# tmtlakmal/acme

Measured on AMD Instinct MI355X. Metric: learner transitions/sec (sample+step) at batch 512, 1/2/4/8 MI355X, higher is better.
Workload: dtype f32 (2xf16 split planes, 3 MFMA terms); 1 GPU; dqn_nature_cnn_prioritized_replay (BASELINE configs[1]); global_batch=512, batch_per_gpu=512, replay_slots=1000000, replay_slots_per_gpu=1000000, obs=uint8[84,84,4], num_actions=18, sampler=prioritized(alpha=0.6), IS beta=0.2, prefetch_size=4, parallelism=dp1

## Files before the change

### acme_amd/_lib.py

```python

from __future__ import annotations

import ctypes
import os
import threading

import torch

_HERE = os.path.dirname(os.path.abspath(__file__))
LIB_PATH = os.environ.get("ACME_LIB_PATH") or os.path.join(_HERE, "libacme_hip.so")

ACME_OK = 0
ACME_ERR_INVALID = -1
ACME_ERR_HIP = -2
ACME_ERR_EMPTY = -3
ACME_ERR_OOM = -4

SEMANTICS_TF = 0
SEMANTICS_JAX = 1

MATMUL_F32 = 0
MATMUL_X6 = 1

MAX_FIELDS = 16
# ... 196 lines not shown
    "acme_replay_update_priorities_gated": (c_i32, [c_vp, c_vp, c_vp, c_i64, c_vp, c_vp]),
    "acme_replay_size": (c_i64, [c_vp]),
    "acme_replay_capacity": (c_i64, [c_vp]),
    "acme_replay_debug_leaves": (c_i32, [c_vp, ctypes.POINTER(c_vp), ctypes.POINTER(c_vp),
                                         ctypes.POINTER(c_vp)]),
    "acme_replay_debug_level": (c_i32, [c_vp, c_i32, ctypes.POINTER(c_vp),
                                        ctypes.POINTER(c_i64), ctypes.POINTER(c_i32)]),
    "acme_replay_storage": (c_i32, [c_vp, c_i32, ctypes.POINTER(c_vp)]),
    "acme_replay_inserted": (c_i64, [c_vp]),
    "acme_replay_restore": (c_i32, [c_vp, c_i64, c_vp]),
    "acme_demo_store_create": (c_i32, [c_i64, c_vp, c_i32, c_vp, c_i64, ctypes.POINTER(c_vp)]),
    "acme_demo_store_destroy": (c_i32, [c_vp]),
    "acme_demo_store_upload": (c_i32, [c_vp, ctypes.POINTER(c_vp)]),
    "acme_demo_mix": (c_i32, [c_vp, c_f64, c_i32, c_f32, c_u64, c_u64, c_i64,
                              ctypes.POINTER(c_vp), c_vp, c_vp, c_vp, c_vp, c_vp, c_vp]),
    "acme_seq_demo_mix": (c_i32, [c_vp, c_f64, c_i64, c_i64, c_u64, c_u64, c_i64,
                                  ctypes.POINTER(c_vp), c_i32, c_vp, c_vp, c_vp, c_vp, c_vp,
                                  c_vp, c_vp, c_vp]),
    "acme_dqn_num_params": (c_i64, [c_vp]),
    "acme_dqn_plane_overflow": (c_i32, [c_vp, ctypes.POINTER(c_i32), c_i32]),
    "acme_dqn_verdict_timeouts": (c_i32, [c_vp, ctypes.POINTER(c_i64)]),
    "acme_dqn_update_rider_launches": (c_i64, [c_vp]),
    "acme_dqn_fused_x2_launches": (c_i64, [c_vp]),
    "acme_dqn_skip_word": (c_i32, [c_vp, ctypes.POINTER(c_vp)]),
    "acme_dqn_set_reissue": (c_i32, [c_vp, c_i32]),
    "acme_dqn_verdicts_issued": (c_i64, [c_vp]),
    "acme_dqn_step_verdict": (c_i32, [c_vp, c_i64, ctypes.POINTER(c_i32)]),
    "acme_dqn_set_data_parallel_gate": (c_i32, [c_vp, c_i32]),
    "acme_dqn_dense_grads_ready": (c_i32, [c_vp, c_vp]),
    "acme_dqn_dp_init": (c_i32, [c_vp, c_vp, c_i32]),
    "acme_dqn_dp_step": (c_i32, [c_vp, ctypes.POINTER(TransitionBatch), ctypes.POINTER(DQNOutputs),
                                 c_vp]),
    "acme_nccl_get_unique_id": (c_i32, [c_vp]),
    "acme_nccl_comm_init": (c_i32, [c_vp, c_i32, c_i32, ctypes.POINTER(c_vp)]),
    "acme_nccl_comm_destroy": (c_i32, [c_vp]),
    "acme_dqn_forward_backward": (c_i32, [c_vp, ctypes.POINTER(TransitionBatch),
                                          ctypes.POINTER(DQNOutputs), c_vp]),
    "acme_dqn_apply": (c_i32, [c_vp, c_vp]),
    "acme_dqn_forward_backward_stage": (c_i32, [c_vp, ctypes.POINTER(TransitionBatch),
                                                ctypes.POINTER(DQNOutputs), c_i32, c_vp]),
    "acme_dqn_grad_split": (c_i32, [c_vp, ctypes.POINTER(c_i64)]),
    "acme_dqn_step": (c_i32, [c_vp, ctypes.POINTER(TransitionBatch), ctypes.POINTER(DQNOutputs),
                              c_vp]),
    "acme_dqn_step_update": (c_i32, [c_vp, ctypes.POINTER(TransitionBatch),
                                     ctypes.POINTER(DQNOutputs), c_vp, c_vp, c_vp, c_vp]),
    "acme_dqn_q_values": (c_i32, [c_vp, c_vp, c_i64, c_i32, c_vp, c_vp]),
# ... 180 lines not shown
```

### acme_amd/csrc/dqn.hip

```cpp
#include <hip/hip_runtime.h>

#include <algorithm>
#include <cmath>
#include <cstring>
#include <string>
#include <vector>

#include "common.h"
#include "conv.h"
#include "rescale.h"
#include "conv_p3.h"
#include "gemm.h"
#include "gemm_p3.h"
#include "gemm_x6.h"
#include "kernels.h"
#include "launch.h"
#include "learner_common.h"
#include "plane_guard.h"
#include "prio_update.h"
#include "profiler.h"
#include "rccl_dyn.h"
#include "torso.h"

using namespace acme;
using namespace acme::conv;
using acme::gemm::launch_gemm;

namespace {

using torso::G1;
constexpr int kFlat = torso::kFlat;
constexpr int kHidden = 512;
constexpr int kObsBytes = 84 * 84 * 4;

struct Layer {
  int in = 0, out = 0;
  int w = -1, b = -1;
// ... 57 lines not shown
  uint16_t *wpl = nullptr, *tpl = nullptr;
  uint16_t* frames = nullptr;
  StepState step;
  hipStream_t side = nullptr;
  hipEvent_t ev[4] = {nullptr, nullptr, nullptr, nullptr};
  float* slab2 = nullptr;
  float* side_slab = nullptr;
  float* tslab = nullptr;
  bool target_dirty = true;
  torso::Plane x1p{}, x2p{}, x3p{}, t1p{}, t2p{}, t3p{}, dzhp{}, dz3p{}, dz2p{}, dz1p{};
  hipEvent_t ev_dense = nullptr;
  void* dp_comm = nullptr;
  int dp_world = 0;
  hipStream_t dp_stream = nullptr;
  hipEvent_t dp_ev[4] = {nullptr, nullptr, nullptr, nullptr};
  double* dp_gmin = nullptr;
  double* loss_part = nullptr;
  bool single_stream = false;
  bool single_role = false;
  bool bk32 = false;
  bool update_rider = true;
  int64_t rider_launches = 0;
  bool head_fuse = true;
  int fuse_x2 = torso::kFuseX2Default;
  int64_t fused_x2_launches = 0;
  bool frames_u8 = true;
  int64_t seq = 0;
  uint32_t* host_verdicts = nullptr;
  uint32_t verdict_seq = 0;
  bool sticky = false;
  bool dp_gate = false;
  int64_t dp_gate_index = -1;
};

namespace {

enum {
  kScX1, kScX2, kScX3, kScT1, kScT2, kScT3, kScDzh, kScDz3, kScDz2, kScDz1,
  kScTransient,
  kScParams = kScTransient, kScTarget,
  kScCount
};
constexpr int64_t kParamAmaxPeriod = 8;
constexpr int kVerdictRing = 64;

int add_tensor(acme_dqn* l, const std::string& name, std::initializer_list<int64_t> shape) {
// ... 3 lines not shown
}

inline torso::Plane WP(const acme_dqn* l, uint16_t* base, int t) {
  return torso::Plane{base + l->tensors[t].offset, l->flat,
                      l->scales + (base == l->tpl ? kScTarget : kScParams)};
}
int convert_frames(acme_dqn* l, const void* obs_a, const void* obs_b, int split, int rows,
                   hipStream_t st) {
  ACME_PROF("frames_f16", st, 0.0, 3.0 * (double)rows * kObsBytes);
  return launch_frames_f16(static_cast<const uint8_t*>(obs_a), static_cast<const uint8_t*>(obs_b),
                           split, rows, kObsBytes, l->frames, st);
}
bool use_p3(const acme_dqn* l) { return l->p3_capable && gemm::use_x6(); }
Gate step_gate(const acme_dqn* l) {
  Gate q;
  q.g = l->guard;
  q.par = (int)(l->seq & 1);
  if (l->dp_gate) q.dp = l->grads + l->dp_gate_index;
  return q;
}
hipStream_t side_stream(const acme_dqn* l) { return prof::enabled() ? nullptr : l->side; }

constexpr int kFcFwdSplits = 8;
constexpr int kHeadFwdSplits = 16;
constexpr int kHeadBwdSplits = 8;

int64_t slab_floats_needed(int B, int A) {
  return std::max<int64_t>({torso::wgrad_slab_floats(), (int64_t)kFcFwdSplits * 2 * B * 2 * kHidden,
                            (int64_t)kHeadFwdSplits * 2 * B * (A + 1),
                            (int64_t)kHeadBwdSplits * (2 * kHidden + 1) * (A + 1)});
}

int slab_reduce(const float* slab, int splits, int64_t count, float* out0, int64_t split_at,
                float* out1, const float* bias, int ncols, int relu, const char* name,
                hipStream_t st) {
  ACME_PROF(name, st, 0.0, 4.0 * (double)(splits + 1) * (double)count);
  return launch_slab_reduce(slab, splits, count, out0, split_at, out1, bias, ncols, relu, st);
}

int adam_range(acme_dqn* l, int64_t off, int64_t n, const Gate& gate, const AdamTail& tail,
               hipStream_t st) {
  const bool jax = l->cfg.semantics == ACME_SEMANTICS_JAX;
  const bool p3 = l->p3_capable;
  return launch_adam(l->params + off, l->grads + off, l->m + off, l->v + off, n,
                     l->cfg.learning_rate, l->cfg.adam_beta1, l->cfg.adam_beta2,
                     l->cfg.adam_epsilon, 0, p3 ? l->wpl + off : nullptr, l->flat, st, jax ? 1 : 0,
// ... 50 lines not shown
  return head_forward(l, prm, rows, hid, q, st);
}

template <int BM>
int fc_fwd_gemm(const acme_dqn* l, const char* name, P3DenseFwd p, int splits,
                hipStream_t st) {
  if (l->single_role) ACME_P3_GEMM(name, BM, 128, 2, 2, 32, p, splits);
  else ACME_P3WS_GEMM(name, BM, 128, 2, 2, 32, p, splits);
  return ACME_OK;
}

int nature_forward_p3(acme_dqn* l, const float* prm, uint16_t* wpl, const torso::Frames& frames,
                      int rows, const torso::Plane& x1, const torso::Plane& x2,
                      const torso::Plane& x3, float* hid, float* q, hipStream_t st,
                      float* slab = nullptr, int keep_x1 = -1, bool defer_head = false,
                      int keep_x2 = -1) {
  if (!slab) slab = l->slab;
  int rc = torso::forward_p3(torso_pweights(l, prm, wpl), frames, rows, torso::PActs{x1, x2, x3}, st, keep_x1, l->bk32, keep_x2);
  if (rc != ACME_OK) return rc;
  {
    P3DenseFwd p;
    const bool tall = rows > 512;
    const bool ttall = rows == 512 && !defer_head;
    const int splits = kFcFwdSplits;
    p.M = rows; p.N = 2 * kHidden; p.K = kFlat; p.k_chunk = chunk_for(kFlat, splits);
    p.a_src = SRC(x3, (int64_t)rows * kFlat); p.ldx = kFlat;
    p.b_src = SRC(WP(l, wpl, l->t_fcw), (int64_t)kFlat * 2 * kHidden); p.slab = slab;
    if (tall) p.stamps = l->stamps;
    rc = tall || ttall ? fc_fwd_gemm<256>(l, ttall ? "fc_fwd_target" : "fc_fwd", p, splits, st)
                       : fc_fwd_gemm<128>(l, "fc_fwd", p, splits, st);
    if (rc != ACME_OK) return rc;
    if (defer_head && l->head_fuse &&
        dqn_head_loss_dz_fusable(kHidden, l->cfg.num_actions, splits, P(l, prm, l->t_vw),
                                 P(l, prm, l->t_aw), P(l, prm, l->t_fcb))) {
      l->step.head_deferred = true;
      l->step.head_splits = splits;
      return ACME_OK;
    }
    ACME_PROF("fc_head_fwd", st, 0.0, 4.0 * (double)rows * 2 * kHidden * (splits + 1));
    return launch_fc_head_forward(slab, splits, rows, kHidden, P(l, prm, l->t_fcb),
                                  P(l, prm, l->t_vw), P(l, prm, l->t_vb), P(l, prm, l->t_aw),
                                  P(l, prm, l->t_ab), l->cfg.num_actions, hid, q, st);
  }
}

template <class In>
int mlp_layer(acme_dqn* l, const float* prm, const Layer& L, const void* a, const void* b,
              int split, int rows, float* y, hipStream_t st) {
  const bool vec = L.in % 4 == 0 && L.out % 4 == 0;
  if (vec) {
    DenseFwd<true, In> p;
    p.M = rows; p.N = L.out; p.K = L.in; p.k_chunk = L.in;
    p.x = static_cast<const typename In::T*>(a); p.x2 = static_cast<const typename In::T*>(b);
// ... 76 lines not shown
                     s.upd_n >= 1 && s.upd_n <= kUpdateRiderMax;
  if (rider) {
    if (plan.after) ACME_HIP_TRY(hipStreamWaitEvent(st, plan.after, 0));
    const RescaleJob job = take_step_rescale(l, true);
    if ((rc = replay_update_prepare(plan.replay, plan.keys, s.upd_prio, s.upd_n, step_gate(l), st,
                                    &job, kUpdateRiderBlocks, &upd)) != ACME_OK)
      return rc;
    l->rider_launches += 1;
    s.update_issued = true;
  }
  rc = torso::backward_p3_conv1(g, s.cur_frames, B, l->dz1p, l->slab, st, sd,
                                rider ? &upd : nullptr);
  if (rider) replay_update_release(plan.replay);
  if (rc != ACME_OK) return rc;
  if (write_back && !rider) {
    s.update_issued = true;
    if (plan.after) ACME_HIP_TRY(hipStreamWaitEvent(st, plan.after, 0));
    const RescaleJob job = take_step_rescale(l, true);
    if ((rc = replay_update_priorities_gated(plan.replay, plan.keys, s.upd_prio, s.upd_n,
                                             step_gate(l), st, &job)) != ACME_OK)
      return rc;
  }
  return torso::backward_p3_join(st, sd);
}

int nature_backward(acme_dqn* l, const StepPlan& plan, const void* o_tm1, int B,
                    hipStream_t st_main, bool join_dense) {
  StepState& s = l->step;
  hipStream_t st = st_main;
  const float* prm = l->params;
  float* gr = l->grads;
  const int A = l->cfg.num_actions;
  const bool p3 = use_p3(l);
  int rc;
  bool loss_sum = false;
  const LossArgs la = s.pending_la;
  if (p3 && s.loss_pending && s.head_deferred) {
    s.loss_pending = s.head_deferred = false;
    loss_sum = true;
    s.loss_nparts = B;
    ACME_PROF("head_loss_dz", st, 0.0, 4.0 * (double)2 * B * 2 * kHidden * (s.head_splits + 1));
    rc = launch_dqn_head_loss_dz(la, l->slab, s.head_splits, kHidden, P(l, prm, l->t_fcb),
                                 P(l, prm, l->t_vw), P(l, prm, l->t_vb), P(l, prm, l->t_aw),
                                 P(l, prm, l->t_ab), l->hid, l->dzhp.p, l->dzhp.stride,
                                 l->dzhp.sc, st,
                                 l->stamps && B <= 4096 ? l->stamps + (int64_t)5 * 4096 * 8 : nullptr);
    if (rc != ACME_OK) return rc;
  } else if (p3 && s.loss_pending) {
    s.loss_pending = false;
    loss_sum = la.loss_part != nullptr;
    s.loss_nparts = dqn_loss_head_dz_blocks(B, kHidden);
    ACME_PROF("loss_head_dz", st, 0.0, 0.0);
    rc = launch_dqn_loss_head_dz(la, l->hid, kHidden, P(l, prm, l->t_vw),
                                 P(l, prm, l->t_aw), l->dzhp.p, l->dzhp.stride, l->dzhp.sc, st);
    if (rc != ACME_OK) return rc;
  } else {
    ACME_PROF("head_dz", st, 0.0, 0.0);
    rc = p3 ? launch_head_dz_planes(l->hid, l->g, l->a_cache, B, kHidden, A, P(l, prm, l->t_vw),
                                    P(l, prm, l->t_aw), l->dzhp.p, l->dzhp.stride, l->dzhp.sc, st)
            : launch_duel_head_dz(l->hid, l->g, l->a_cache, B, kHidden, A, P(l, prm, l->t_vw),
                                  P(l, prm, l->t_aw), l->dzh, st);
    if (rc != ACME_OK) return rc;
  }
  const bool fork = p3 && side_stream(l);
  float* hslab = fork ? l->side_slab : l->slab;
  if (fork) {
    ACME_HIP_TRY(hipEventRecord(l->ev[2], st_main));
    ACME_HIP_TRY(hipStreamWaitEvent(l->side, l->ev[2], 0));
    st = l->side;
  }
  if (p3 && plan.replay) {
    s.upd_prio = la.prio;
    s.upd_n = B;
  }
  const bool sum_in_scatter = loss_sum;
  {
    DuelHeadWgrad p;
    p.M = 2 * kHidden; p.N = A + 1; p.K = B; p.k_chunk = chunk_for(B, kHeadBwdSplits);
    p.A = A; p.h = l->hid; p.g = l->g; p.act = l->a_cache; p.slab = hslab;
    ACME_GEMM("head_wgrad", 64, 32, 2, 1, 16, 1, p, kHeadBwdSplits);
    ACME_PROF("head_wgrad_scatter", st, 0.0, 0.0);
    rc = launch_duel_head_grad_scatter(
        hslab, kHeadBwdSplits, kHidden, A, Pm(l, gr, l->t_vw), Pm(l, gr, l->t_vb),
        Pm(l, gr, l->t_aw), Pm(l, gr, l->t_ab), st, sum_in_scatter ? la.loss_part : nullptr,
        s.loss_nparts, la.mean_over, la.loss);
    if (rc != ACME_OK) return rc;
  }
  if (p3) {
    {
      P3DenseWgrad p;
      p.M = kFlat; p.N = 2 * kHidden; p.K = B; p.k_chunk = B;
      p.a_src = SRC(l->x3p, (int64_t)B * kFlat); p.ldx = kFlat;
      p.b_src = SRC(l->dzhp, (int64_t)B * 2 * kHidden); p.out = Pm(l, gr, l->t_fcw);
      p.bias_out = Pm(l, gr, l->t_fcb);
      ACME_P3_GEMM("fc_wgrad", 128, 128, 2, 2, 16, p, 1);
    }
    if (fork) {
      ACME_HIP_TRY(hipEventRecord(l->ev[3], l->side));
      st = st_main;
    }
    {
      P3DenseDgrad p;
      p.M = B; p.N = kFlat; p.K = 2 * kHidden; p.k_chunk = p.K;
      p.a_src = SRC(l->dzhp, (int64_t)B * 2 * kHidden);
      p.b_src = SRC(WP(l, l->wpl, l->t_fcw), (int64_t)kFlat * 2 * kHidden); p.xprev = CP(l->x3p);
      p.ldx = kFlat; p.dx = PP(l->dz3p);
      if (l->single_role) ACME_P3G_GEMM("fc_dgrad", 128, 128, 2, 2, 32, 3, p, 1);
      else ACME_P3WS_GEMM("fc_dgrad", 128, 128, 2, 2, 32, p, 1);
    }
    if (fork && join_dense) ACME_HIP_TRY(hipStreamWaitEvent(st_main, l->ev[3], 0));
    if (fork) s.dense_ev = l->ev[3];
    return ACME_OK;
  }
  {
    DenseWgrad<true> p;
    p.M = kFlat; p.N = 2 * kHidden; p.K = B; p.k_chunk = B;
    p.x = l->x3; p.ldx = kFlat; p.dz = l->dzh; p.out = Pm(l, gr, l->t_fcw);
    p.bias_out = Pm(l, gr, l->t_fcb);
    ACME_GEMM("fc_wgrad", 128, 128, 2, 2, 16, 1, p, 1);
  }
  {
    DenseDgrad<true> p;
    p.M = B; p.N = kFlat; p.K = 2 * kHidden; p.k_chunk = p.K;
    p.dz = l->dzh; p.w = P(l, prm, l->t_fcw); p.xprev = l->x3; p.ldx = kFlat; p.dx = l->dz3;
    ACME_GEMM("fc_dgrad", 64, 128, 2, 2, 16, 1, p, 1);
  }
  return ACME_OK;
}

template <class In>
int mlp_wgrad(acme_dqn* l, const Layer& L, const void* x, const float* dz, int B, float* dw,
              float* db, hipStream_t st) {
  if (L.in % 4 == 0 && L.out % 4 == 0) {
    DenseWgrad<true, In> p;
    p.M = L.in; p.N = L.out; p.K = B; p.k_chunk = B;
    p.x = static_cast<const typename In::T*>(x); p.ldx = L.in; p.dz = dz; p.out = dw;
// ... 67 lines not shown
}

extern "C" {

int acme_dqn_create(const acme_dqn_config* cfg, acme_dqn** out) {
  ACME_CHECK_ARG(cfg && out, "null argument");
  ACME_CHECK_ARG(cfg->num_actions >= 1 && cfg->num_actions <= 63, "num_actions must be in [1, 63]");
  ACME_CHECK_ARG(cfg->max_batch >= 1 && cfg->max_batch <= 65536, "max_batch must be in [1, 65536]");
  ACME_CHECK_ARG(cfg->network == ACME_NET_NATURE_DQN || cfg->network == ACME_NET_MLP,
                 "unknown network kind %d", cfg->network);
  ACME_CHECK_ARG(cfg->obs_dtype == ACME_OBS_U8_SCALED || cfg->obs_dtype == ACME_OBS_F32,
                 "unknown observation dtype %d", cfg->obs_dtype);
  ACME_CHECK_ARG(cfg->huber_loss_parameter >= 0.f, "quadratic_linear_boundary must be >= 0.");
  ACME_CHECK_ARG(cfg->target_update_period >= 1, "target_update_period must be >= 1");
  ACME_CHECK_ARG(cfg->semantics == ACME_SEMANTICS_TF || cfg->semantics == ACME_SEMANTICS_JAX,
                 "unknown learner semantics %d", cfg->semantics);
  acme_dqn* l = new acme_dqn();
  l->cfg = *cfg;
  l->single_stream = tune_variant("SIDE") == 1;
  l->single_role = tune_variant("WSN") == 1;
  l->bk32 = tune_variant("BK32") == 1;
  l->update_rider = tune_variant("UPDATE_RIDER", kUpdateRiderDefault) != 0;
  l->head_fuse = tune_variant("HEAD_FUSE", 1) != 0;
  l->fuse_x2 = tune_variant("FUSE_X2", torso::kFuseX2Default) & 3;
  l->stamps_on = tune_variant("STAMPS") == 1;
  const int A = cfg->num_actions;
  const int B = cfg->max_batch;
  int rc = ACME_OK;
  auto fail = [&](int code) {
    acme_dqn_destroy(l);
    return code;
  };
  if ((rc = guard_create(l)) != ACME_OK) return fail(rc);
  if (hipHostMalloc(reinterpret_cast<void**>(&l->host_verdicts), kVerdictRing * sizeof(uint32_t),
                    hipHostMallocCoherent | hipHostMallocMapped) != hipSuccess)
    return fail((set_error("step guard allocation failed"), ACME_ERR_HIP));
  for (int i = 0; i < kVerdictRing; ++i) l->host_verdicts[i] = 0xFFFFFFFFu;
  if (cfg->network == ACME_NET_NATURE_DQN) {
    l->t_c1w = add_tensor(l, "atari_torso/conv2_d/w", {8, 8, 4, 32});
    l->t_c1b = add_tensor(l, "atari_torso/conv2_d/b", {32});
    l->t_c2w = add_tensor(l, "atari_torso/conv2_d_1/w", {4, 4, 32, 64});
    l->t_c2b = add_tensor(l, "atari_torso/conv2_d_1/b", {64});
    l->t_c3w = add_tensor(l, "atari_torso/conv2_d_2/w", {3, 3, 64, 64});
    l->t_c3b = add_tensor(l, "atari_torso/conv2_d_2/b", {64});
    l->t_fcw = add_tensor(l, "duelling_q_network/hidden/w", {kFlat, 2 * kHidden});
    l->t_fcb = add_tensor(l, "duelling_q_network/hidden/b", {2 * kHidden});
// ... 172 lines not shown
int acme_dqn_guard_state(acme_dqn* l, int64_t* out4) {
  ACME_CHECK_ARG(l && out4 && l->guard, "null argument");
  StepGuard g;
  if (int rc = read_guard(l, &g)) return rc;
  out4[0] = g.applied;
  out4[1] = g.skipped;
  out4[2] = g.last;
  out4[3] = g.qv;
  return ACME_OK;
}

int acme_dqn_verdict_timeouts(acme_dqn* l, int64_t* out) {
  ACME_CHECK_ARG(l && out, "null argument");
  *out = 0;
  if (!l->guard) return ACME_OK;
  StepGuard g;
  if (int rc = read_guard(l, &g)) return rc;
  *out = g.vtimeout;
  return ACME_OK;
}

int64_t acme_dqn_update_rider_launches(const acme_dqn* l) { return l ? l->rider_launches : 0; }
int64_t acme_dqn_fused_x2_launches(const acme_dqn* l) { return l ? l->fused_x2_launches : 0; }

int acme_dqn_set_reissue(acme_dqn* l, int32_t enable) {
  ACME_CHECK_ARG(l, "null learner");
  l->sticky = enable != 0 && l->p3_capable;
  return ACME_OK;
}

int64_t acme_dqn_verdicts_issued(const acme_dqn* l) { return l ? (int64_t)l->verdict_seq : 0; }

int acme_dqn_step_verdict(const acme_dqn* l, int64_t seq, int32_t* state) {
  ACME_CHECK_ARG(l && state && seq >= 0, "bad argument");
  *state = -1;
  if (!l->host_verdicts || seq >= (int64_t)l->verdict_seq) return ACME_OK;
  ACME_CHECK_ARG(seq + kVerdictRing >= (int64_t)l->verdict_seq,
                 "verdict %lld is older than the ring's %d", (long long)seq, kVerdictRing);
  const uint32_t v =
      __atomic_load_n(l->host_verdicts + (seq & (kVerdictRing - 1)), __ATOMIC_ACQUIRE);
  if ((v >> 1) == ((uint32_t)seq & 0x7fffffffu)) *state = (int32_t)(v & 1u);
  return ACME_OK;
}

int acme_dqn_set_applied_steps(acme_dqn* l, int64_t n) {
  ACME_CHECK_ARG(l && l->guard && n >= 0, "bad argument");
// ... 518 lines not shown
```

### acme_amd/csrc/kernels.hip

```cpp
#include "kernels.h"
#include "rescale.h"

#include "conv.h"
#include "gemm_p3.h"
#include "gemm_x6.h"

#include <hip/hip_runtime.h>

#include <algorithm>
#include <cmath>

#include "common.h"
#include "detmath.h"

namespace acme {
namespace {

__global__ void __launch_bounds__(256) duel_head_finish_kernel(const float* __restrict__ slab,
                                                               int splits, int rows, int A,
                                                               const float* __restrict__ bv,
                                                               const float* __restrict__ ba,
                                                               float* __restrict__ q) {
  const int lane = threadIdx.x & 63;
  const int row = blockIdx.x * 4 + (threadIdx.x >> 6);
  if (row >= rows) return;
  const int N = A + 1;
  float* qr = q + (size_t)row * A;
  float v = 0.f;
  for (int s = 0; s < splits; ++s) v += slab[((size_t)s * rows + row) * N + A];
  v += bv[0];
  float first = 0.f, part = 0.f;
  for (int j = lane; j < A; j += 64) {
    float acc = 0.f;
    for (int s = 0; s < splits; ++s) acc += slab[((size_t)s * rows + row) * N + j];
    acc += ba[j];
    if (j == lane) {
// ... 113 lines not shown
                                    float* __restrict__ dzh, uint16_t* __restrict__ planes,
                                    int64_t pstride, gemm::PScale* sc) {
  const int64_t i = (int64_t)blockIdx.x * blockDim.x + threadIdx.x;
  if (i >= (int64_t)B * 2 * H) return;
  const int b = (int)(i / (2 * H));
  const int k = (int)(i - (int64_t)b * 2 * H);
  const float gb = g[b];
  float d;
  if (k < H) {
    d = gb * wv[k];
  } else {
    const float* row = wa + (size_t)(k - H) * A;
    const float inv_a = 1.f / (float)A;
    const int ab = a[b];
    float s = 0.f;
    for (int j = 0; j < A; ++j) s = fmaf(gb * ((j == ab ? 1.f : 0.f) - inv_a), row[j], s);
    d = s;
  }
  const float z = h[i] > 0.f ? d : 0.f;
  if (planes) gemm::Planes{planes, pstride, sc}.put(i, z);
  else dzh[i] = z;
}

__device__ __forceinline__ void loss_sum_block(const double* __restrict__ part, int64_t n,
                                               int mean_over, float* __restrict__ loss) {
  __shared__ double red[4];
  const int tid = threadIdx.x, lane = tid & 63, wave = tid >> 6;
  double s = 0.0;
  for (int64_t i = tid; i < n; i += 256) s += part[i];
#pragma unroll
  for (int o = 32; o > 0; o >>= 1) s += __shfl_xor(s, o, 64);
  if (lane == 0) red[wave] = s;
  __syncthreads();
  if (tid == 0) loss[0] = (float)((((red[0] + red[1]) + red[2]) + red[3]) / (double)mean_over);
}

__global__ void __launch_bounds__(256) duel_head_grad_scatter_kernel(
    const float* __restrict__ slab, int splits, int H, int A, float* __restrict__ dwv,
    float* __restrict__ dbv, float* __restrict__ dwa, float* __restrict__ dba,
    const double* __restrict__ part, int64_t nparts, int mean_over, float* __restrict__ loss) {
  if (part && blockIdx.x == gridDim.x - 1) {
    loss_sum_block(part, nparts, mean_over, loss);
    return;
  }
  const int N = A + 1;
  const int64_t count = (int64_t)(2 * H + 1) * N;
  const int64_t e = (int64_t)blockIdx.x * blockDim.x + threadIdx.x;
  if (e >= count) return;
  const int k = (int)(e / N), n = (int)(e - (int64_t)k * N);
  const bool value_w = k < H && n == A, adv_w = k >= H && k < 2 * H && n < A, bias = k == 2 * H;
  if (!(value_w || adv_w || bias)) return;
  float s = 0.f;
  for (int sp = 0; sp < splits; ++sp) s += slab[(size_t)sp * count + e];
  if (value_w) dwv[k] = s;
  else if (adv_w) dwa[(size_t)(k - H) * A + n] = s;
  else if (n == A) dbv[0] = s;
  else dba[n] = s;
}

__global__ void onehot_dq_kernel(const float* __restrict__ g, const int32_t* __restrict__ a,
                                 int B, int A, float* __restrict__ dz) {
  const int i = blockIdx.x * blockDim.x + threadIdx.x;
  if (i >= B * A) return;
  const int b = i / A, j = i - b * A;
  dz[i] = j == a[b] ? g[b] : 0.f;
// ... 1282 lines not shown
         reinterpret_cast<uintptr_t>(fcb) % 16 == 0;
}

int launch_dqn_head_loss_dz(const LossArgs& args, const float* slab, int splits, int H,
                            const float* fcb, const float* wv, const float* bv, const float* wa,
                            const float* ba, float* hid, uint16_t* planes, int64_t pstride,
                            gemm::PScale* sc, hipStream_t st, uint64_t* stamps) {
  ACME_CHECK_ARG(dqn_head_loss_dz_fusable(H, args.A, splits, wv, wa, fcb) && args.loss_part &&
                     planes && sc && args.B >= 1,
                 "bad fused head / loss / head dZ arguments");
  if (splits == 8)
    dqn_head_loss_dz_kernel<8, 18><<<(unsigned)args.B, 256, 0, st>>>(args, slab, fcb, wv, bv, wa, ba,
                                                                   hid, planes, pstride, sc, stamps);
  else
    dqn_head_loss_dz_kernel<4, 18><<<(unsigned)args.B, 256, 0, st>>>(args, slab, fcb, wv, bv, wa, ba,
                                                                   hid, planes, pstride, sc, stamps);
  ACME_LAUNCH_CHECK();
  return ACME_OK;
}

__global__ void __launch_bounds__(256) dqn_loss_sum_kernel(const double* __restrict__ part,
                                                           int64_t n, int mean_over,
                                                           float* __restrict__ loss) {
  loss_sum_block(part, n, mean_over, loss);
}

int launch_dqn_loss_sum(const double* part, int64_t n, int mean_over, float* loss, hipStream_t st) {
  ACME_CHECK_ARG(part && loss && n >= 1 && mean_over >= 1, "bad loss sum args");
  dqn_loss_sum_kernel<<<1, 256, 0, st>>>(part, n, mean_over, loss);
  ACME_LAUNCH_CHECK();
  return ACME_OK;
}

int launch_dqn_loss_head_dz(const LossArgs& args, const float* h, int H, const float* wv,
                            const float* wa, uint16_t* planes, int64_t pstride, gemm::PScale* sc,
                            hipStream_t st) {
  ACME_CHECK_ARG(args.B >= 1 && args.A >= 1 && h && wv && wa && planes && sc,
                 "bad loss / head dZ args");
  const int per = 2 * H / 8;
  ACME_CHECK_ARG(H % 8 == 0 && per >= 32 && 256 % per == 0, "hidden size %d: 2H/8 must divide 256", H);
  ACME_CHECK_ARG(reinterpret_cast<uintptr_t>(wv) % 16 == 0, "wv must be 16-byte aligned");
  const int64_t nb = ceil_div((int64_t)args.B * per, 256);
  dqn_loss_head_dz_kernel<<<(unsigned)(args.loss_part ? nb : nb + 1), 256, 0, st>>>(
      args, h, H, wv, wa, planes, pstride, sc);
  ACME_LAUNCH_CHECK();
  return ACME_OK;
}
// ... 296 lines not shown
```

### acme_amd/native.py

```python

from __future__ import annotations

import ctypes
from typing import Dict, List, Optional, Sequence, Tuple

import numpy as np
import torch

from acme_amd import _lib
from acme_amd._lib import check, lib, ptr, stream_ptr

SAMPLER_UNIFORM = 0
SAMPLER_PRIORITIZED = 1


class NativeReplay:

    def __init__(self, capacity: int, field_bytes: Sequence[int], prioritized: bool,
                 priority_exponent: float = 0.6, seed: int = 1234, device=None):
        _lib.require_gpu()
        if len(field_bytes) > _lib.MAX_FIELDS:
            raise ValueError(f"at most {_lib.MAX_FIELDS} flattened fields per item")
        cfg = _lib.ReplayConfig()
        cfg.capacity = int(capacity)
# ... 585 lines not shown
        self.semantics = semantics
        self.network = network
        self.num_actions = int(num_actions)
        self.max_batch = int(max_batch)
        self._create(cfg, device)
        self.num_params = int(lib().acme_dqn_num_params(self._h))
        d = self.device
        self.loss = torch.zeros(1, dtype=torch.float32, device=d)
        self.td_error = torch.zeros(max_batch, dtype=torch.float32, device=d)
        self.priorities = torch.zeros(max_batch, dtype=torch.float64, device=d)

    def guard_state(self) -> Dict[str, int]:
        g = super().guard_state()
        t = ctypes.c_int64()
        check(lib().acme_dqn_verdict_timeouts(self._h, ctypes.byref(t)), "dqn verdict_timeouts")
        g["verdict_timeouts"] = int(t.value)
        return g

    def update_rider_launches(self) -> int:
        return int(lib().acme_dqn_update_rider_launches(self._h))

    def fused_x2_launches(self) -> int:
        return int(lib().acme_dqn_fused_x2_launches(self._h))

    @property
    def skip_word(self) -> Optional[int]:
        p = ctypes.c_void_p()
        check(lib().acme_dqn_skip_word(self._h, ctypes.byref(p)), "dqn skip_word")
        return p.value

    def set_reissue(self, enable: bool) -> None:
        check(lib().acme_dqn_set_reissue(self._h, 1 if enable else 0), "dqn set_reissue")

    @property
    def verdicts_issued(self) -> int:
        return int(lib().acme_dqn_verdicts_issued(self._h))

    def step_verdict(self, seq: int) -> Optional[bool]:
        v = ctypes.c_int32(-1)
        check(lib().acme_dqn_step_verdict(self._h, int(seq), ctypes.byref(v)), "dqn step_verdict")
        return None if v.value < 0 else bool(v.value)

    def set_data_parallel_gate(self, enable: bool) -> None:
        check(lib().acme_dqn_set_data_parallel_gate(self._h, 1 if enable else 0), "dqn dp gate")

    def _batch(self, o_tm1, a_tm1, r_t, d_t, o_t, probabilities, global_min_probability=None,
# ... 532 lines not shown
```

### include/acme_hip.h

```cpp
#ifndef ACME_HIP_H_
#define ACME_HIP_H_

#include <stdint.h>

#ifdef __cplusplus
extern "C" {
#endif

typedef enum acme_status {
  ACME_OK = 0,
  ACME_ERR_INVALID = -1,
  ACME_ERR_HIP = -2,
  ACME_ERR_EMPTY = -3,
  ACME_ERR_OOM = -4
} acme_status;

const char* acme_last_error(void);

int acme_tune_set(const char* key, int32_t value);
const char* acme_version(void);
const char* acme_target_arch(void);

int acme_event_create(void** ev);
int acme_event_destroy(void* ev);
// ... 177 lines not shown

int acme_dqn_create(const acme_dqn_config* cfg, acme_dqn** out);
int acme_dqn_destroy(acme_dqn* l);
int64_t acme_dqn_num_params(const acme_dqn* l);
int64_t acme_dqn_flat_size(const acme_dqn* l);
int32_t acme_dqn_num_tensors(const acme_dqn* l);
int acme_dqn_tensor_info(const acme_dqn* l, int32_t i, int64_t* offset, int64_t* numel,
                         int32_t* ndim, int64_t* shape4, const char** name);

int acme_dqn_bind(acme_dqn* l, float* params, float* target, float* grads, float* adam_m,
                  float* adam_v);
int acme_dqn_params_changed(acme_dqn* l);
int acme_dqn_plane_overflow(acme_dqn* l, int32_t* overflow, int32_t reset);
int64_t acme_dqn_skipped_steps(const acme_dqn* l);
int acme_dqn_guard_state(acme_dqn* l, int64_t* out4);
int acme_dqn_set_applied_steps(acme_dqn* l, int64_t n);
int acme_dqn_skip_word(const acme_dqn* l, const uint32_t** out);
int acme_dqn_set_data_parallel_gate(acme_dqn* l, int32_t enable);
int acme_dqn_set_reissue(acme_dqn* l, int32_t enable);
int acme_dqn_verdict_timeouts(acme_dqn* l, int64_t* out);
int64_t acme_dqn_verdicts_issued(const acme_dqn* l);
int64_t acme_dqn_update_rider_launches(const acme_dqn* l);
int64_t acme_dqn_fused_x2_launches(const acme_dqn* l);
int acme_dqn_step_verdict(const acme_dqn* l, int64_t seq, int32_t* state);
int acme_dqn_scale_state(const acme_dqn* l, float* out, int32_t capacity, int32_t* count);
int acme_dqn_set_scale_state(acme_dqn* l, const float* in, int32_t count);

typedef struct acme_transition_batch {
  const void* o_tm1;
  const int32_t* a_tm1;
  const float* r_t;
  const float* d_t;
  const void* o_t;
  const double* probabilities;
  int64_t batch;
  const double* global_min_probability;
  int64_t mean_over;
  const uint16_t* obs_f16;
  void* inputs_event;
} acme_transition_batch;

typedef struct acme_dqn_outputs {
  float* loss;
  float* td_error;
  double* priorities;
  float* q_tm1;
// ... 379 lines not shown
```

Measured before the change: 1.152 million transitions/s.

## Fuse dueling head weight-gradient into fc_wgrad GEMM as rider blocks; split tall fc_fwd fewer ways

Introduces a HeadWgradRider that computes the dueling head's value/advantage weight and bias gradients, plus the loss sum, in extra workgroups appended to the fc_wgrad P3 GEMM launch. This replaces the separate split-K head_wgrad GEMM and its scatter kernel. The head backward and fc_dgrad are also restructured into helpers, and the whole dense wgrad chain now runs on the side stream. Separately, tall deferred-head forward passes use 4 K-splits with 128-wide tiles instead of 8 splits with 256-wide tiles. Both paths are on by default behind tune flags, and the rider adds a register-heavy 18-accumulator path inside the GEMM kernel.

After: 1.158 million transitions/s (median of 6 runs). No clear change (+0.5%).

```diff
diff --git a/acme_amd/_lib.py b/acme_amd/_lib.py
--- a/acme_amd/_lib.py
+++ b/acme_amd/_lib.py
@@ -242,6 +242,7 @@
     "acme_dqn_verdict_timeouts": (c_i32, [c_vp, ctypes.POINTER(c_i64)]),
     "acme_dqn_update_rider_launches": (c_i64, [c_vp]),
     "acme_dqn_fused_x2_launches": (c_i64, [c_vp]),
+    "acme_dqn_head_rider_launches": (c_i64, [c_vp]),
     "acme_dqn_skip_word": (c_i32, [c_vp, ctypes.POINTER(c_vp)]),
     "acme_dqn_set_reissue": (c_i32, [c_vp, c_i32]),
     "acme_dqn_verdicts_issued": (c_i64, [c_vp]),
diff --git a/acme_amd/csrc/dqn.hip b/acme_amd/csrc/dqn.hip
--- a/acme_amd/csrc/dqn.hip
+++ b/acme_amd/csrc/dqn.hip
@@ -13,6 +13,7 @@
 #include "gemm.h"
 #include "gemm_p3.h"
 #include "gemm_x6.h"
+#include "head_rider.h"
 #include "kernels.h"
 #include "launch.h"
 #include "learner_common.h"
@@ -116,6 +117,9 @@
   bool update_rider = true;
   int64_t rider_launches = 0;
   bool head_fuse = true;
+  bool fc_split4 = true;
+  bool head_rider = true;
+  int64_t head_rider_launches = 0;
   int fuse_x2 = torso::kFuseX2Default;
   int64_t fused_x2_launches = 0;
   bool frames_u8 = true;
@@ -165,6 +169,7 @@
 hipStream_t side_stream(const acme_dqn* l) { return prof::enabled() ? nullptr : l->side; }
 
 constexpr int kFcFwdSplits = 8;
+constexpr int kFcFwdSplitsTall = 4;
 constexpr int kHeadFwdSplits = 16;
 constexpr int kHeadBwdSplits = 8;
 
@@ -261,13 +266,15 @@
     P3DenseFwd p;
     const bool tall = rows > 512;
     const bool ttall = rows == 512 && !defer_head;
-    const int splits = kFcFwdSplits;
+    const bool half = tall && defer_head && l->fc_split4;
+    const int splits = half ? kFcFwdSplitsTall : kFcFwdSplits;
     p.M = rows; p.N = 2 * kHidden; p.K = kFlat; p.k_chunk = chunk_for(kFlat, splits);
     p.a_src = SRC(x3, (int64_t)rows * kFlat); p.ldx = kFlat;
     p.b_src = SRC(WP(l, wpl, l->t_fcw), (int64_t)kFlat * 2 * kHidden); p.slab = slab;
     if (tall) p.stamps = l->stamps;
-    rc = tall || ttall ? fc_fwd_gemm<256>(l, ttall ? "fc_fwd_target" : "fc_fwd", p, splits, st)
-                       : fc_fwd_gemm<128>(l, "fc_fwd", p, splits, st);
+    rc = (tall && !half) || ttall
+             ? fc_fwd_gemm<256>(l, ttall ? "fc_fwd_target" : "fc_fwd", p, splits, st)
+             : fc_fwd_gemm<128>(l, "fc_fwd", p, splits, st);
     if (rc != ACME_OK) return rc;
     if (defer_head && l->head_fuse &&
         dqn_head_loss_dz_fusable(kHidden, l->cfg.num_actions, splits, P(l, prm, l->t_vw),
@@ -390,6 +397,58 @@
       return rc;
   }
   return torso::backward_p3_join(st, sd);
+}
+
+int head_wgrad(acme_dqn* l, const LossArgs& la, const double* part, int B, float* hslab,
+               hipStream_t st) {
+  const int A = l->cfg.num_actions;
+  float* gr = l->grads;
+  DuelHeadWgrad p;
+  p.M = 2 * kHidden; p.N = A + 1; p.K = B; p.k_chunk = chunk_for(B, kHeadBwdSplits);
+  p.A = A; p.h = l->hid; p.g = l->g; p.act = l->a_cache; p.slab = hslab;
+  ACME_GEMM("head_wgrad", 64, 32, 2, 1, 16, 1, p, kHeadBwdSplits);
+  ACME_PROF("head_wgrad_scatter", st, 0.0, 0.0);
+  return launch_duel_head_grad_scatter(hslab, kHeadBwdSplits, kHidden, A, Pm(l, gr, l->t_vw),
+                                       Pm(l, gr, l->t_vb), Pm(l, gr, l->t_aw), Pm(l, gr, l->t_ab),
+                                       st, part, l->step.loss_nparts, la.mean_over, la.loss);
+}
+
+int dense_wgrads_p3(acme_dqn* l, const StepPlan& plan, const LossArgs& la, const double* part,
+                    int B, float* hslab, hipStream_t st) {
+  float* gr = l->grads;
+  HeadWgradArgs ra;
+  ra.h = l->hid; ra.g = l->g; ra.act = l->a_cache;
+  ra.B = B; ra.A = l->cfg.num_actions; ra.H = kHidden;
+  ra.dwv = Pm(l, gr, l->t_vw); ra.dbv = Pm(l, gr, l->t_vb);
+  ra.dwa = Pm(l, gr, l->t_aw); ra.dba = Pm(l, gr, l->t_ab);
+  ra.part = part; ra.nparts = l->step.loss_nparts; ra.mean_over = la.mean_over; ra.loss = la.loss;
+  const bool rider = l->head_rider && !plan.calibrating && HeadWgradRider::fits(ra);
+  int rc;
+  if (!rider && (rc = head_wgrad(l, la, part, B, hslab, st)) != ACME_OK) return rc;
+  P3DenseWgrad p;
+  p.M = kFlat; p.N = 2 * kHidden; p.K = B; p.k_chunk = B;
+  p.a_src = SRC(l->x3p, (int64_t)B * kFlat); p.ldx = kFlat;
+  p.b_src = SRC(l->dzhp, (int64_t)B * 2 * kHidden); p.out = Pm(l, gr, l->t_fcw);
+  p.bias_out = Pm(l, gr, l->t_fcb);
+  if (rider) {
+    l->head_rider_launches += 1;
+    ACME_LAUNCH_GEMM("fc_wgrad", ACME_MNK_FLOPS(p), gemm::p3_peak_tflops<decltype(p)>(),
+                     (gemm::launch_gemm_p3_rider<128, 128, 2, 2, 16, HeadWgradRider>(p, 1, ra, st)));
+  } else {
+    ACME_P3_GEMM("fc_wgrad", 128, 128, 2, 2, 16, p, 1);
+  }
+  return ACME_OK;
+}
+
+int fc_dgrad_p3(acme_dqn* l, int B, hipStream_t st) {
+  P3DenseDgrad p;
+  p.M = B; p.N = kFlat; p.K = 2 * kHidden; p.k_chunk = p.K;
+  p.a_src = SRC(l->dzhp, (int64_t)B * 2 * kHidden);
+  p.b_src = SRC(WP(l, l->wpl, l->t_fcw), (int64_t)kFlat * 2 * kHidden); p.xprev = CP(l->x3p);
+  p.ldx = kFlat; p.dx = PP(l->dz3p);
+  if (l->single_role) ACME_P3G_GEMM("fc_dgrad", 128, 128, 2, 2, 32, 3, p, 1);
+  else ACME_P3WS_GEMM("fc_dgrad", 128, 128, 2, 2, 32, p, 1);
+  return ACME_OK;
 }
 
 int nature_backward(acme_dqn* l, const StepPlan& plan, const void* o_tm1, int B,
@@ -430,56 +489,27 @@
                                   P(l, prm, l->t_aw), l->dzh, st);
     if (rc != ACME_OK) return rc;
   }
-  const bool fork = p3 && side_stream(l);
-  float* hslab = fork ? l->side_slab : l->slab;
-  if (fork) {
-    ACME_HIP_TRY(hipEventRecord(l->ev[2], st_main));
-    ACME_HIP_TRY(hipStreamWaitEvent(l->side, l->ev[2], 0));
-    st = l->side;
-  }
   if (p3 && plan.replay) {
     s.upd_prio = la.prio;
     s.upd_n = B;
   }
-  const bool sum_in_scatter = loss_sum;
-  {
-    DuelHeadWgrad p;
-    p.M = 2 * kHidden; p.N = A + 1; p.K = B; p.k_chunk = chunk_for(B, kHeadBwdSplits);
-    p.A = A; p.h = l->hid; p.g = l->g; p.act = l->a_cache; p.slab = hslab;
-    ACME_GEMM("head_wgrad", 64, 32, 2, 1, 16, 1, p, kHeadBwdSplits);
-    ACME_PROF("head_wgrad_scatter", st, 0.0, 0.0);
-    rc = launch_duel_head_grad_scatter(
-        hslab, kHeadBwdSplits, kHidden, A, Pm(l, gr, l->t_vw), Pm(l, gr, l->t_vb),
-        Pm(l, gr, l->t_aw), Pm(l, gr, l->t_ab), st, sum_in_scatter ? la.loss_part : nullptr,
-        s.loss_nparts, la.mean_over, la.loss);
-    if (rc != ACME_OK) return rc;
-  }
+  const double* part = loss_sum ? la.loss_part : nullptr;
   if (p3) {
-    {
-      P3DenseWgrad p;
-      p.M = kFlat; p.N = 2 * kHidden; p.K = B; p.k_chunk = B;
-      p.a_src = SRC(l->x3p, (int64_t)B * kFlat); p.ldx = kFlat;
-      p.b_src = SRC(l->dzhp, (int64_t)B * 2 * kHidden); p.out = Pm(l, gr, l->t_fcw);
-      p.bias_out = Pm(l, gr, l->t_fcb);
-      ACME_P3_GEMM("fc_wgrad", 128, 128, 2, 2, 16, p, 1);
-    }
+    const bool fork = side_stream(l) != nullptr;
+    hipStream_t ws = fork ? l->side : st_main;
     if (fork) {
-      ACME_HIP_TRY(hipEventRecord(l->ev[3], l->side));
-      st = st_main;
-    }
-    {
-      P3DenseDgrad p;
-      p.M = B; p.N = kFlat; p.K = 2 * kHidden; p.k_chunk = p.K;
-      p.a_src = SRC(l->dzhp, (int64_t)B * 2 * kHidden);
-      p.b_src = SRC(WP(l, l->wpl, l->t_fcw), (int64_t)kFlat * 2 * kHidden); p.xprev = CP(l->x3p);
-      p.ldx = kFlat; p.dx = PP(l->dz3p);
-      if (l->single_role) ACME_P3G_GEMM("fc_dgrad", 128, 128, 2, 2, 32, 3, p, 1);
-      else ACME_P3WS_GEMM("fc_dgrad", 128, 128, 2, 2, 32, p, 1);
-    }
+      ACME_HIP_TRY(hipEventRecord(l->ev[2], st_main));
+      ACME_HIP_TRY(hipStreamWaitEvent(l->side, l->ev[2], 0));
+    }
+    if ((rc = dense_wgrads_p3(l, plan, la, part, B, fork ? l->side_slab : l->slab, ws)) != ACME_OK)
+      return rc;
+    if (fork) ACME_HIP_TRY(hipEventRecord(l->ev[3], l->side));
+    if ((rc = fc_dgrad_p3(l, B, st_main)) != ACME_OK) return rc;
     if (fork && join_dense) ACME_HIP_TRY(hipStreamWaitEvent(st_main, l->ev[3], 0));
     if (fork) s.dense_ev = l->ev[3];
     return ACME_OK;
   }
+  if ((rc = head_wgrad(l, la, part, B, l->slab, st)) != ACME_OK) return rc;
   {
     DenseWgrad<true> p;
     p.M = kFlat; p.N = 2 * kHidden; p.K = B; p.k_chunk = B;
@@ -593,6 +623,8 @@
   l->bk32 = tune_variant("BK32") == 1;
   l->update_rider = tune_variant("UPDATE_RIDER", kUpdateRiderDefault) != 0;
   l->head_fuse = tune_variant("HEAD_FUSE", 1) != 0;
+  l->fc_split4 = tune_variant("FC_SPLIT4", 1) != 0;
+  l->head_rider = tune_variant("HEAD_RIDER", 1) != 0;
   l->fuse_x2 = tune_variant("FUSE_X2", torso::kFuseX2Default) & 3;
   l->stamps_on = tune_variant("STAMPS") == 1;
   const int A = cfg->num_actions;
@@ -811,6 +843,7 @@
 
 int64_t acme_dqn_update_rider_launches(const acme_dqn* l) { return l ? l->rider_launches : 0; }
 int64_t acme_dqn_fused_x2_launches(const acme_dqn* l) { return l ? l->fused_x2_launches : 0; }
+int64_t acme_dqn_head_rider_launches(const acme_dqn* l) { return l ? l->head_rider_launches : 0; }
 
 int acme_dqn_set_reissue(acme_dqn* l, int32_t enable) {
   ACME_CHECK_ARG(l, "null learner");
diff --git a/acme_amd/csrc/head_rider.h b/acme_amd/csrc/head_rider.h
--- /dev/null
+++ b/acme_amd/csrc/head_rider.h
@@ -0,0 +1,134 @@
+#pragma once
+
+#include <hip/hip_runtime.h>
+
+#include <cstdint>
+
+namespace acme {
+
+__device__ __forceinline__ void loss_sum_block(const double* __restrict__ part, int64_t n,
+                                               int mean_over, float* __restrict__ loss,
+                                               double* red) {
+  const int tid = threadIdx.x, lane = tid & 63, wave = tid >> 6;
+  double s = 0.0;
+  for (int64_t i = tid; i < n; i += 256) s += part[i];
+#pragma unroll
+  for (int o = 32; o > 0; o >>= 1) s += __shfl_xor(s, o, 64);
+  if (lane == 0) red[wave] = s;
+  __syncthreads();
+  if (tid == 0) loss[0] = (float)((((red[0] + red[1]) + red[2]) + red[3]) / (double)mean_over);
+}
+
+constexpr int kHeadRiderMaxA = 18;
+
+struct HeadWgradArgs {
+  const float* h = nullptr;
+  const float* g = nullptr;
+  const int32_t* act = nullptr;
+  int B = 0, A = 0, H = 0;
+  float *dwv = nullptr, *dbv = nullptr, *dwa = nullptr, *dba = nullptr;
+  const double* part = nullptr;
+  int64_t nparts = 0;
+  int mean_over = 1;
+  float* loss = nullptr;
+};
+
+struct HeadWgradRider {
+  using Args = HeadWgradArgs;
+  static constexpr int kThreads = 256;
+  static constexpr int kUnits = 8;
+  static constexpr int kLanes = kThreads / kUnits;
+  static constexpr int kLdsBytes = 4 * kUnits * (kHeadRiderMaxA + 1) * (int)sizeof(float);
+  static __host__ __device__ __forceinline__ int groups(const Args& a) {
+    return 2 * a.H / kUnits;
+  }
+  static __host__ __device__ __forceinline__ int blocks(const Args& a) {
+    return (groups(a) + 2 + 7) & ~7;
+  }
+  static __host__ bool fits(const Args& a) {
+    return a.A >= 1 && a.A <= kHeadRiderMaxA && a.H >= 32 && a.H % 32 == 0 && a.B >= 1;
+  }
+  static __device__ __forceinline__ float coef(float gb, int ab, int n, float inv_a) {
+    return gb * ((n == ab ? 1.f : 0.f) - inv_a);
+  }
+  static __device__ __forceinline__ void run(const Args& a, uint8_t* lds, int wg) {
+    constexpr int NA = kHeadRiderMaxA;
+    const int G = groups(a);
+    const int tid = threadIdx.x, lane = tid & 63, wave = tid >> 6;
+    const float inv_a = 1.f / (float)a.A;
+    float* red = reinterpret_cast<float*>(lds);
+    if (wg < G) {
+      const int u = tid & (kUnits - 1), bl = tid / kUnits;
+      const int c = kUnits * ((wg & 7) * (G >> 3) + (wg >> 3)) + u;
+      const bool adv = c >= a.H;
+      const float* hc = a.h + c;
+      const int64_t ld = 2 * (int64_t)a.H;
+      float acc[NA];
+#pragma unroll
+      for (int n = 0; n < NA; ++n) acc[n] = 0.f;
+      if (adv) {
+#pragma unroll 4
+        for (int b = bl; b < a.B; b += kLanes) {
+          const float hv = hc[b * ld], gb = a.g[b];
+          const int ab = a.act[b];
+#pragma unroll
+          for (int n = 0; n < NA; ++n) acc[n] = fmaf(coef(gb, ab, n, inv_a), hv, acc[n]);
+        }
+      } else {
+#pragma unroll 4
+        for (int b = bl; b < a.B; b += kLanes) acc[0] = fmaf(a.g[b], hc[b * ld], acc[0]);
+      }
+#pragma unroll
+      for (int n = 0; n < NA; ++n) {
+        if (adv || n == 0) {
+          float s = acc[n];
+#pragma unroll
+          for (int o = kUnits; o < 64; o <<= 1) s += __shfl_xor(s, o, 64);
+          if (lane < kUnits) red[(wave * kUnits + u) * NA + n] = s;
+        }
+      }
+      __syncthreads();
+      if (tid < kUnits * NA) {
+        const int uu = tid / NA, n = tid - uu * NA;
+        const int cc = c - u + uu;
+        const float s = ((red[(0 * kUnits + uu) * NA + n] + red[(1 * kUnits + uu) * NA + n]) +
+                         red[(2 * kUnits + uu) * NA + n]) +
+                        red[(3 * kUnits + uu) * NA + n];
+        if (adv) {
+          if (n < a.A) a.dwa[(int64_t)(cc - a.H) * a.A + n] = s;
+        } else if (n == 0) {
+          a.dwv[cc] = s;
+        }
+      }
+    } else if (wg == G) {
+      float acc[NA + 1];
+#pragma unroll
+      for (int n = 0; n <= NA; ++n) acc[n] = 0.f;
+      for (int b = tid; b < a.B; b += kThreads) {
+        const float gb = a.g[b];
+        const int ab = a.act[b];
+#pragma unroll
+        for (int n = 0; n < NA; ++n) acc[n] += coef(gb, ab, n, inv_a);
+        acc[NA] += gb;
+      }
+#pragma unroll
+      for (int n = 0; n <= NA; ++n) {
+        float s = acc[n];
+#pragma unroll
+        for (int o = 1; o < 64; o <<= 1) s += __shfl_xor(s, o, 64);
+        if (lane == 0) red[wave * (NA + 1) + n] = s;
+      }
+      __syncthreads();
+      if (tid <= NA) {
+        const float s = ((red[tid] + red[(NA + 1) + tid]) + red[2 * (NA + 1) + tid]) +
+                        red[3 * (NA + 1) + tid];
+        if (tid == NA) a.dbv[0] = s;
+        else if (tid < a.A) a.dba[tid] = s;
+      }
+    } else if (wg == G + 1 && a.part) {
+      loss_sum_block(a.part, a.nparts, a.mean_over, a.loss, reinterpret_cast<double*>(lds));
+    }
+  }
+};
+
+}
diff --git a/acme_amd/csrc/kernels.hip b/acme_amd/csrc/kernels.hip
--- a/acme_amd/csrc/kernels.hip
+++ b/acme_amd/csrc/kernels.hip
@@ -12,6 +12,7 @@
 
 #include "common.h"
 #include "detmath.h"
+#include "head_rider.h"
 
 namespace acme {
 namespace {
@@ -171,25 +172,14 @@
   else dzh[i] = z;
 }
 
-__device__ __forceinline__ void loss_sum_block(const double* __restrict__ part, int64_t n,
-                                               int mean_over, float* __restrict__ loss) {
-  __shared__ double red[4];
-  const int tid = threadIdx.x, lane = tid & 63, wave = tid >> 6;
-  double s = 0.0;
-  for (int64_t i = tid; i < n; i += 256) s += part[i];
-#pragma unroll
-  for (int o = 32; o > 0; o >>= 1) s += __shfl_xor(s, o, 64);
-  if (lane == 0) red[wave] = s;
-  __syncthreads();
-  if (tid == 0) loss[0] = (float)((((red[0] + red[1]) + red[2]) + red[3]) / (double)mean_over);
-}
 
 __global__ void __launch_bounds__(256) duel_head_grad_scatter_kernel(
     const float* __restrict__ slab, int splits, int H, int A, float* __restrict__ dwv,
     float* __restrict__ dbv, float* __restrict__ dwa, float* __restrict__ dba,
     const double* __restrict__ part, int64_t nparts, int mean_over, float* __restrict__ loss) {
+  __shared__ double red[4];
   if (part && blockIdx.x == gridDim.x - 1) {
-    loss_sum_block(part, nparts, mean_over, loss);
+    loss_sum_block(part, nparts, mean_over, loss, red);
     return;
   }
   const int N = A + 1;
@@ -1518,7 +1508,8 @@
 __global__ void __launch_bounds__(256) dqn_loss_sum_kernel(const double* __restrict__ part,
                                                            int64_t n, int mean_over,
                                                            float* __restrict__ loss) {
-  loss_sum_block(part, n, mean_over, loss);
+  __shared__ double red[4];
+  loss_sum_block(part, n, mean_over, loss, red);
 }
 
 int launch_dqn_loss_sum(const double* part, int64_t n, int mean_over, float* loss, hipStream_t st) {
diff --git a/acme_amd/native.py b/acme_amd/native.py
--- a/acme_amd/native.py
+++ b/acme_amd/native.py
@@ -631,6 +631,9 @@
 
     def fused_x2_launches(self) -> int:
         return int(lib().acme_dqn_fused_x2_launches(self._h))
+
+    def head_rider_launches(self) -> int:
+        return int(lib().acme_dqn_head_rider_launches(self._h))
 
     @property
     def skip_word(self) -> Optional[int]:
diff --git a/include/acme_hip.h b/include/acme_hip.h
--- a/include/acme_hip.h
+++ b/include/acme_hip.h
@@ -223,6 +223,7 @@
 int64_t acme_dqn_verdicts_issued(const acme_dqn* l);
 int64_t acme_dqn_update_rider_launches(const acme_dqn* l);
 int64_t acme_dqn_fused_x2_launches(const acme_dqn* l);
+int64_t acme_dqn_head_rider_launches(const acme_dqn* l);
 int acme_dqn_step_verdict(const acme_dqn* l, int64_t seq, int32_t* state);
 int acme_dqn_scale_state(const acme_dqn* l, float* out, int32_t capacity, int32_t* count);
 int acme_dqn_set_scale_state(acme_dqn* l, const float* in, int32_t count);
```
